# GrafikXxxxxxxYyyyyyyyyyy/StableDiffusion

Hardware: AMD Instinct MI355X
Metric: denoise-loop latents/s (512px, 50-step DDIM, batch 4) (higher is better)
Workload: dtype f16; 1 GPU; SD1.5 512x512, 50-step DDIM, batch 4/GPU, CFG on (UNet batch 8), UNet + VAE decode HIP kernels; global_batch=4, parallelism=dp1

## Files before the change

include/sd_engine.h:

```cpp
#ifndef SD_ENGINE_H
#define SD_ENGINE_H

#include <stdint.h>

#ifdef __cplusplus
extern "C" {
#endif

#define SD_OK 0
#define SD_ERR_INVALID 1
#define SD_ERR_STATE 2
#define SD_ERR_HIP 3
#define SD_ERR_UNSUPPORTED 4

#define SD_DTYPE_F16 0
#define SD_DTYPE_F32 1

#define SD_MAX_BLOCKS 4

typedef struct sd_unet_config {
    int32_t in_channels;
    int32_t out_channels;
    int32_t num_blocks;
    int32_t block_out_channels[SD_MAX_BLOCKS];
// ... 205 lines not shown

int sd_probe_mfma(int iters, float* tflops, void* stream);
int sd_probe_copy(int64_t bytes, int iters, float* gbs, void* stream);
int sd_probe_lds_dma(int64_t region_bytes, int passes, int depth, int shared, float* gbs, void* stream);

int sd_igemm_force(int variant, int splits);
int sd_igemm_plan(const int* geom, const int* flags, int64_t* out, char* name);

int sd_op_conv2d(const void* x_nhwc, const void* w_oihw, const void* bias, const void* rowadd,
                 const void* res_nhwc, void* y_nhwc, int N, int H, int W, int Cin, int Cout,
                 int ksize, int stride, int upsample2x, int geglu, void* stream);
int sd_op_conv2d_ex(const void* x_nhwc, const void* w_oihw, const void* bias, const void* rowadd,
                    const void* res_nhwc, void* y_nhwc, int N, int H, int W, int Cin, int Cout, int ksize,
                    int stride, int upsample2x, int geglu, int64_t ldx, int64_t ldres, int64_t ldy, int pad, int act,
                    float acc_scale, float bias_scale, int gn_groups, int* ran, void* stream);
int sd_op_conv3x3_small_cout(const void* x_nhwc, const void* w_oihw, const void* bias, void* y_nchw, int N, int H,
                             int W, int Cin, int Cout, void* stream);
int sd_op_conv2d_groupnorm(const void* x_nhwc, const void* w_oihw, const void* bias, const void* rowadd,
                           const void* res_nhwc, void* y_conv_nhwc, const void* gamma, const void* beta,
                           void* y_gn_nhwc, int N, int H, int W, int Cin, int Cout, int ksize, int stride,
                           int upsample2x, int groups, float eps, int silu, int* stats_from_epilogue, void* stream);
int sd_op_groupnorm_conv2d(const void* x_nhwc, const void* gamma, const void* beta, int groups, float eps, int silu,
                           const void* w_oihw, const void* bias, const void* rowadd, const void* res_nhwc, void* y_nhwc,
                           int N, int H, int W, int Cin, int Cout, int ksize, int iters, float* ms_per_launch, int* fused,
                           void* stream);
int sd_op_unet_conv_in(const void* x_nchw, const void* w_oihw, const void* bias, void* y_nhwc, float* gn_summaries, int groups,
                       int N, int Cin, int H, int W, int Cout, int iters, float* ms_per_launch, void* stream);
int sd_op_unet_conv_out(const void* x_nhwc, const void* gamma, const void* beta, int groups, float eps, int silu,
                        const void* w_oihw, const void* bias, void* y_nchw, int N, int H, int W, int C, int Cout, int iters,
                        float* ms_per_launch, void* stream);
// ... 79 lines not shown
```

stablediffusion_amd/_lib.py:

```python
from __future__ import annotations

import ctypes as C
import os

_HERE = os.path.dirname(os.path.abspath(__file__))
LIB_PATH = os.path.join(_HERE, "libsd_engine.so")

SD_MAX_BLOCKS = 4
SD_STEP_MAX_SLOTS = 4
SD_STEP_MAX_WRITES = 2
SD_DTYPE_F16 = 0
SD_DTYPE_F32 = 1


class SdUNetConfig(C.Structure):
    _fields_ = [
        ("in_channels", C.c_int32),
        ("out_channels", C.c_int32),
        ("num_blocks", C.c_int32),
        ("block_out_channels", C.c_int32 * SD_MAX_BLOCKS),
        ("down_block_has_attn", C.c_int32 * SD_MAX_BLOCKS),
        ("up_block_has_attn", C.c_int32 * SD_MAX_BLOCKS),
        ("num_heads", C.c_int32 * SD_MAX_BLOCKS),
        ("transformer_layers", C.c_int32 * SD_MAX_BLOCKS),
# ... 172 lines not shown
    "sd_images_to_uint8": (_I, [_P, _P, _I, _I, _I, _I, _P]),
    "sd_cfg_linear_step": (_I, [_P, _P, _P, _I64, _F, _F, _F, _F, _F, _F, _P]),
    "sd_cfg_rescale_linear_step": (_I, [_P, _P, _P, _I, _I64, _F, _F, _F, _F, _F, _F, _F, _P, _P]),
    "sd_lcm_step": (_I, [_P, _I, _P, _P, _P, _I64, _F, _F, _F, _F, _F, _P]),
    "sd_sched_affine_step": (_I, [_P, _I, _P, _P, _P, _I64, _I64, _F, C.POINTER(SdStepPlan), _P]),
    "sd_igemm_force": (_I, [_I, _I]),
    "sd_igemm_plan": (_I, [C.POINTER(_I), C.POINTER(_I), C.POINTER(_I64), C.c_char_p]),
    "sd_probe_mfma": (_I, [_I, C.POINTER(_F), _P]),
    "sd_probe_lds_dma": (_I, [_I64, _I, _I, _I, C.POINTER(_F), _P]),
    "sd_probe_copy": (_I, [_I64, _I, C.POINTER(_F), _P]),
    "sd_prof_enable": (_I, [_I]),
    "sd_prof_collect": (_I, [C.POINTER(SdProfEntry), _I, C.POINTER(_I)]),
    "sd_op_conv2d": (_I, [_P, _P, _P, _P, _P, _P, _I, _I, _I, _I, _I, _I, _I, _I, _I, _P]),
    "sd_op_conv2d_ex": (_I, [_P, _P, _P, _P, _P, _P, _I, _I, _I, _I, _I, _I, _I, _I, _I, _I64, _I64, _I64, _I, _I, _F, _F, _I,
                             C.POINTER(_I), _P]),
    "sd_op_conv3x3_small_cout": (_I, [_P, _P, _P, _P, _I, _I, _I, _I, _I, _P]),
    "sd_op_conv2d_groupnorm": (_I, [_P, _P, _P, _P, _P, _P, _P, _P, _P, _I, _I, _I, _I, _I, _I, _I, _I, _I, _F, _I,
                                    C.POINTER(_I), _P]),
    "sd_op_groupnorm_conv2d": (_I, [_P, _P, _P, _I, _F, _I, _P, _P, _P, _P, _P, _I, _I, _I, _I, _I, _I, _I, C.POINTER(_F),
                                    C.POINTER(_I), _P]),
    "sd_op_unet_conv_in": (_I, [_P, _P, _P, _P, _P, _I, _I, _I, _I, _I, _I, _I, C.POINTER(_F), _P]),
    "sd_op_unet_conv_out": (_I, [_P, _P, _P, _I, _F, _I, _P, _P, _P, _I, _I, _I, _I, _I, _I, C.POINTER(_F), _P]),
    "sd_op_ffn_geglu": (_I, [_P, _P, _P, _F, _P, _P, _P, _P, _P, _I, _I, _I, C.POINTER(_F), C.POINTER(_I), _P]),
    "sd_op_linear_rowstats": (_I, [_P, _P, _P, _P, _P, _P, _I, _I, _I, C.POINTER(_I), C.POINTER(_I), C.POINTER(_I), _P]),
    "sd_op_ln_linear": (_I, [_P, _P, _I, _I, _P, _P, _F, _P, _P, _P, _I, _I, _I, _I, _I, _F, C.POINTER(_I), _P]),
    "sd_op_ln_ffn_geglu": (_I, [_P, _P, _I, _I, _P, _P, _F, _P, _P, _P, _P, _P, _I, _I, C.POINTER(_I), _P]),
    "sd_op_fold_linear": (_I, [_P, _P, _P, _P, _P, _P, _I, _I, _I, _P]),
    "sd_op_ffn_geglu_proj_out": (_I, [_P, _P, _P, _P, _F, _P, _P, _P, _P, _P, _P, _P, _P, C.POINTER(_I), _I, _I, _I,
                                      C.POINTER(_I), _P]),
    "sd_bench_conv2d": (_I, [_P, _P, _P, _I, _I, _I, _I, _I, _I, _I, _I, _I, _I, C.POINTER(_F), _P]),
# ... 61 lines not shown
```

stablediffusion_amd/csrc/capi.cpp:

```cpp
#include <cmath>
#include <cstdio>
#include <new>

#include "model.h"
#include <cstdlib>

using namespace sd;

struct sd_unet { UNet impl; explicit sd_unet(const sd_unet_config& c) : impl(c) {} };
struct sd_vae { VAE impl; explicit sd_vae(const sd_vae_config& c) : impl(c) {} };
struct sd_clip { CLIP impl; explicit sd_clip(const sd_clip_config& c) : impl(c) {} };
struct sd_clip_vision { CLIPVision impl; explicit sd_clip_vision(const sd_clip_vision_config& c) : impl(c) {} };
struct sd_controlnet {
    ControlNet impl;
    sd_controlnet(const sd_unet_config& c, int cc) : impl(c, cc) {}
};
struct sd_ip_adapter {
    IPAdapter impl;
    sd_ip_adapter(const sd_unet_config& c, const sd_ip_projection_config& p) : impl(c, p) {}
    ~sd_ip_adapter() { if (impl.attached) impl.attached->set_ip_adapter(nullptr); }
};

namespace {

// ... 1690 lines not shown
    WeightStore ws;
    const int64_t so[2] = {O, J}, si[2] = {J, K}, sbo[1] = {O}, sbi[1] = {J};
    ws.declare("o.weight", {O, J}); ws.declare("o.bias", {O});
    ws.declare("i.weight", {J, K}); ws.declare("i.bias", {J});
    int rc;
    if ((rc = ws.set("o.weight", w_outer, so, 2, 0)) || (rc = ws.set("o.bias", b_outer, sbo, 1, 1)) ||
        (rc = ws.set("i.weight", w_inner, si, 2, 0)) || (rc = ws.set("i.bias", b_inner, sbi, 1, 1))) return rc;
    ConvW f;
    if ((rc = ws.fold_linear("o", "i", &f))) return rc;
    SD_HIP_CHECK(hipMemcpy(w_folded, f.w, (size_t)O * f.K * sizeof(half_t), hipMemcpyDeviceToDevice));
    SD_HIP_CHECK(hipMemcpy(b_folded, f.bias, (size_t)O * sizeof(float), hipMemcpyDeviceToDevice));
    SD_HIP_CHECK(hipDeviceSynchronize());
    return SD_OK;
}

int sd_op_ffn_geglu_proj_out(const void* x_in, const void* t3, const void* ln_gamma, const void* ln_beta, float ln_eps,
                             const void* w1, const void* b1, const void* w2, const void* b2, const void* w_po,
                             const void* b_po, void* y, float* gn_summaries, int* gn_rows, int M, int C, int imgs, int* fused,
                             void* stream) {
    if (!x_in || !t3 || !ln_gamma || !ln_beta || !w1 || !b1 || !w2 || !b2 || !w_po || !b_po || !y || M < 1 || C < 64 ||
        C % 64 != 0 || imgs < 1 || M % imgs != 0 || ln_eps != 1e-5f) {
        set_error("sd_op_ffn_geglu_proj_out: bad arguments (C % 64, M % imgs, ln_eps = 1e-5: the transformer's)"); return SD_ERR_INVALID;
    }
    hipStream_t s = static_cast<hipStream_t>(stream);
    SD_HIP_CHECK(hipStreamSynchronize(s));
    const int G = 32;
    WeightStore ws;
    const int64_t C8 = 8L * C, C4 = 4L * C;
    const int64_t s1[2] = {C8, C}, s2[2] = {C, C4}, so[2] = {C, C}, sc[1] = {C}, s8[1] = {C8};
    ws.declare("norm3.weight", {C}); ws.declare("norm3.bias", {C});
// ... 50 lines not shown
```

stablediffusion_amd/csrc/engine.h:

```cpp
#pragma once
#include <map>
#include <string>
#include <unordered_map>
#include <vector>

#include "kernels.h"

namespace sd {

struct View {
    half_t* p = nullptr;
    long ld = 0;
    int C = 0;
    View() {}
    View(half_t* p_, long ld_, int C_) : p(p_), ld(ld_), C(C_) {}
    View slice(int c0, int c) const { return View(p + c0, ld, c); }
};

class Arena {
  public:
    ~Arena();
    int reserve(size_t bytes);
    void begin(bool dry) { dry_ = dry; off_ = 0; if (dry) peak_ = 0; }
    void* alloc(size_t bytes);
// ... 6 lines not shown
    bool dry() const { return dry_; }
    bool overflow() const { return overflow_; }

  private:
    char* base_ = nullptr;
    size_t cap_ = 0, off_ = 0, peak_ = 0;
    bool dry_ = false, overflow_ = false;
};

struct ConvW {
    half_t* w = nullptr;
    float* bias = nullptr;
    int cin = 0, cout = 0, ks = 1;
    long K = 0;
    float* wsum = nullptr;
};
struct RowStat {
    float* p = nullptr;
    int parts = 0;
    int width = 0;
};
struct GnStatBuf {
    float* buf = nullptr;
    GnStats st;
};
struct ConvFuse {
    const RowStat* ln_in = nullptr;
    float ln_eps = 0.f;
    RowStat* stat_out = nullptr;
    GnStatBuf* gn_out = nullptr;
    int gn_groups = 0;
    const struct NormW* gn_in = nullptr;
    GnStats gn_in_stats;
    int gn_in_groups = 0;
    float gn_in_eps = 0.f;
    int gn_in_silu = 0;
    float acc_scale = 1.f, bias_scale = 1.f;
    int tile_variant = -1, tile_splits = 0;
};
struct NormW {
    float* gamma = nullptr;
    float* beta = nullptr;
    float* gb = nullptr;
    int C = 0;
};

struct RawTensor {
    std::vector<int64_t> shape;
    half_t* dev = nullptr;
    long numel = 0;
};

class WeightStore {
  public:
    ~WeightStore();
    void declare(const std::string& key, std::vector<int64_t> shape);
    int set(const std::string& key, const void* data, const int64_t* shape, int ndim, int dtype);
    bool complete(std::string* missing) const;
    const RawTensor* raw(const std::string& key) const;
    int pack_conv(const std::string& prefix, ConvW* out, bool has_bias = true);
    int pack_rows(const std::vector<std::string>& weight_keys, const std::vector<std::string>& bias_keys,
                  ConvW* out);
    int pack_geglu(const std::string& prefix, ConvW* out);
    int pack_norm(const std::string& prefix, NormW* out);
    int fold_ln(ConvW* w, const NormW& ln, int rows_scaled, float row_scale);
    int fold_linear(const std::string& outer, const std::string& inner, ConvW* out);
    void free_raw();
    void* dmalloc(size_t bytes);
    int64_t packed_bytes() const { return packed_bytes_; }

    std::vector<std::string> order;
    std::unordered_map<std::string, RawTensor> tensors;

  private:
    int host_floats(const std::string& key, std::vector<float>* out) const;
// ... 48 lines not shown
```

stablediffusion_amd/csrc/igemm2.hip:

```cpp
#include <atomic>
#include <cstdlib>
#include <mutex>

#include "kernels.h"

namespace sd {
namespace {

constexpr int BK = 64;
constexpr int kMaxLnParts = 20;
template <int N>
__device__ __forceinline__ void wait_vmcnt() {
    static_assert(N >= 0 && N <= 63, "vmcnt is a 6-bit field");
    asm volatile("s_waitcnt vmcnt(%0)" ::"n"(N) : "memory");
}
template <int PER, int YMAX>
__device__ __forceinline__ void wait_stages(int y) {
    if constexpr (YMAX == 0) {
        wait_vmcnt<0>();
    } else {
        if (y >= YMAX) wait_vmcnt<PER * YMAX>();
        else wait_stages<PER, YMAX - 1>(y);
    }
}
// ... 975 lines not shown
}

template <int BN>
int launch_halo(const IGemmParams& p, float* partial, int splits, hipStream_t s) {
    if (p.gni_part) {
        if (p.gni_groups < 1 || p.gni_groups > 32 || 512 % p.gni_groups != 0 || p.Cin % p.gni_groups != 0 || !p.gni_gb) {
            set_error("conv3x3_halo_kernel: fused GroupNorm needs 1..32 groups dividing 512 and the packed affine");
            return 1;
        }
        return launch_halo_t<BN, true, false>(p, partial, splits, s);
    }
    if constexpr (BN == 160) {
        if (p.gnstat_out && splits <= 1) return launch_halo_t<BN, false, false>(p, partial, splits, s);
    }
    return launch_halo_t<BN, false, true>(p, partial, splits, s);
}

template <int BM, int BN, int WM, int WN, int STAGES, bool PW, bool STAG, int BKT>
int launch_v2p(const IGemmParams& p, float* partial, int splits, hipStream_t s) {
    constexpr size_t lds = IGemm2Lds<BM, BN, STAGES, BKT>::TOTAL;
    static_assert(lds <= 160 * 1024, "LDS budget");
    static PerDeviceOnce attr_once;
    if (attr_once.first()) {
        SD_HIP_CHECK(hipFuncSetAttribute(reinterpret_cast<const void*>(&igemm2_kernel<BM, BN, WM, WN, STAGES, PW, STAG, BKT>),
                                         hipFuncAttributeMaxDynamicSharedMemorySize, (int)lds));
    }
    const int tiles = cdiv(p.M, BM) * cdiv(p.Cout, BN);
    const int nk = p.K / BKT;
    const int per = cdiv(nk, splits);
    const int eff_splits = cdiv(nk, per);
// ... 192 lines not shown
    }
    route();
    pl.variant = v;
    pl.splits = sp;
    pl.partial_floats = sp > 1 ? (long)sp * p.M * p.Cout : 0;
    if (p.geglu && (!is_ws(v) || pg_k320) && !forced && pgemm_geglu_supported(p)) pl.kind = kKindPgemmGeglu;
    else if ((v == kReg || (kVariants[v].reg_alt && g3_auto && !forced)) && sp <= 1 && igemm3_supported(p)) pl.kind = kReg;
    else pl.kind = v == kReg ? kRegFallback : v;
    const Variant& t = kVariants[pl.kind == kKindPgemmGeglu ? v : pl.kind];
    pl.bm = t.bm; pl.bn = t.bn;
    if (pl.kind == kKindPgemmGeglu) snprintf(pl.name, sizeof(pl.name), "geglu_persist_kernel");
    else snprintf(pl.name, sizeof(pl.name), t.name, p.KS == 1 && p.stride == 1 && p.up == 0 ? "true" : "false");
    return pl;
}

IGemmLaunchNote igemm2_last_launch() { return t_note; }

int igemm2_max_ln_parts() { return kMaxLnParts; }

int launch_igemm2(const IGemmParams& p, float* partial, hipStream_t s, const IGemmPlan* plan) {
    t_note = IGemmLaunchNote();
    if (p.ln_stat && (p.ln_parts < 1 || p.ln_parts > kMaxLnParts)) {
        set_error("igemm2: ln_parts " + std::to_string(p.ln_parts) + " outside 1.." + std::to_string(kMaxLnParts) +
                  " (row-statistics parts a folded LayerNorm reads per row)");
        return 1;
    }
    IGemmParams q = p;
    IGemmPlan own;
    if (!plan || (plan->splits > 1 && !partial)) {
        q.rowstat_out = nullptr; q.gnstat_out = nullptr;
// ... 11 lines not shown
```

stablediffusion_amd/csrc/kernels.h:

```cpp
#pragma once
#include "common.h"

namespace sd {

struct IGemmParams {
    const half_t* x; long ldx;
    const half_t* w;
    const float* bias;
    const float* rowadd; int rowadd_ld;
    const half_t* res; long ldres;
    half_t* y; long ldy;
    int N, H, W, Cin;
    int OH, OW, Cout;
    int KS, stride, pad, up;
    int M, K;
    int geglu;
    int mfast = 0;
    int act = 0;
    float* rowstat_out = nullptr;
    int rowstat_parts = 0;
    const float* ln_stat = nullptr;
    int ln_parts = 0, ln_C = 0, ln_part_w = 0;
    float ln_eps = 0.f;
    const float* ln_wsum = nullptr;
// ... 28 lines not shown
struct IGemmPlan {
    int kind = kKindIgemm1;
    int variant = -1;
    int splits = 1;
    long partial_floats = 0;
    int bm = 0, bn = 0;
    bool rowstats = false;
    int rs_parts = 1, rs_part_w = 0;
    bool gnstats = false;
    int gn_rows = 0;
    bool scales_ok = false;
    char name[64] = "";
};
IGemmPlan igemm2_plan(IGemmParams& p, const IGemmRequest& rq = IGemmRequest());
int launch_igemm2(const IGemmParams& p, float* partial, hipStream_t s, const IGemmPlan* plan = nullptr);
int igemm2_max_ln_parts();
struct IGemmLaunchNote {
    int splits = 1;
    int reducer = 0;
};
IGemmLaunchNote igemm2_last_launch();
bool igemm3_supported(const IGemmParams& p);
int launch_igemm3(const IGemmParams& p, int mfast, hipStream_t s);
constexpr int kWeightRowPad = 256;
bool wsgemm_supported(const IGemmParams& p);
int wsgemm_rowstat_parts(const IGemmParams& p);
int launch_wsgemm(const IGemmParams& p, hipStream_t s);
bool pgemm_geglu_supported(const IGemmParams& p);
int launch_pgemm_geglu(const IGemmParams& p, hipStream_t s);

// ... 184 lines not shown
```

stablediffusion_amd/csrc/misc.hip:

```cpp
#include <cstdint>
#include <cstdlib>
#include <map>
#include <mutex>
#include <utility>

#include "kernels.h"

namespace sd {
namespace {

__device__ __forceinline__ void sinusoid_pair(float t, int f, int half, float shift, float* sn, float* cs) {
    const float freq = __expf(-9.210340371976184f * (float)f / ((float)half - shift));
    const float ang = t * freq;
    sincosf(ang, sn, cs);
}

__global__ void sinusoid_kernel(const float* __restrict__ t, int t_stride, float* __restrict__ out, int count,
                                int dim, int flip, float shift, long out_ld) {
    const int half = dim >> 1;
    const int i = blockIdx.x * blockDim.x + threadIdx.x;
    if (i >= count * half) return;
    const int b = i / half, f = i - b * half;
    float sn, cs;
    sinusoid_pair(t[(long)b * t_stride], f, half, shift, &sn, &cs);
// ... 203 lines not shown
    if (kq < (long)KH * KW * I) {
        int ci, tap;
        if (I % 64 == 0) {
            const int slab = (int)(kq >> 6), cl = (int)(kq & 63);
            const int cs = slab / (KH * KW);
            tap = slab - cs * (KH * KW);
            ci = cs * 64 + cl;
        } else {
            ci = (int)(kq % I);
            tap = (int)(kq / I);
        }
        const int kh = tap / KW, kw = tap - kh * KW;
        val = w[((o * I + ci) * KH + kh) * KW + kw];
    }
    wp[i] = val;
}

__global__ void cfg_duplicate_kernel(const half_t* __restrict__ lat, half_t* __restrict__ out, long n,
                                     float scale) {
    const long i = (long)blockIdx.x * blockDim.x + threadIdx.x;
    if (i >= n) return;
    const half_t v = (half_t)((float)lat[i] * scale);
    out[i] = v;
    out[n + i] = v;
}
constexpr int RD_PER_THREAD = 4;
constexpr int RD_UNITS = 256 * RD_PER_THREAD;
struct RowDupDev {
    const uint4* src[kRowDupMax];
    uint4* dst[kRowDupMax];
// ... 652 lines not shown
    SD_HIP_CHECK(hipGetLastError());
    return 0;
}
int launch_conv3x3_small_cout(const half_t* x, long ldx, const half_t* w, long K, const float* bias, half_t* y_nchw,
                              int N, int H, int W, int Cin, int Cout, hipStream_t s) {
    if (Cout < 1 || Cout > 4 || Cin % 64 != 0 || K != 9L * Cin) { set_error("conv3x3_small_cout: Cout in 1..4, Cin % 64 == 0"); return 1; }
    const long tiles = (long)N * ((H + CO_TH - 1) / CO_TH) * ((W + CO_TW - 1) / CO_TW);
    if (tiles == 0) return 0;
    hipLaunchKernelGGL(conv3x3_small_cout_kernel<4>, dim3((unsigned)tiles), dim3(256), 0, s, x, ldx, w, K, bias, y_nchw, N, H, W,
                       Cin, Cout);
    SD_HIP_CHECK(hipGetLastError());
    return 0;
}
int launch_pack_conv(const half_t* w, half_t* wp, int O, int I, int KH, int KW, long Kpad, hipStream_t s) {
    hipLaunchKernelGGL(pack_conv_kernel, grid1d((long)O * Kpad), dim3(256), 0, s, w, wp, O, I, KH, KW, Kpad);
    SD_HIP_CHECK(hipGetLastError());
    return 0;
}
int launch_cfg_duplicate(const half_t* lat, half_t* out, long n, float scale, hipStream_t s) {
    hipLaunchKernelGGL(cfg_duplicate_kernel, grid1d(n), dim3(256), 0, s, lat, out, n, scale);
    SD_HIP_CHECK(hipGetLastError());
    return 0;
}
int launch_row_dup(const RowDupSeg* segs, int count, hipStream_t s) {
    if (count < 0 || count > kRowDupMax) { set_error("row_dup: too many segments"); return 1; }
    RowDupDev p;
    int blocks = 0, k = 0;
    for (int i = 0; i < count; ++i) {
        const RowDupSeg& g = segs[i];
        if (g.rows <= 0 || g.row_bytes <= 0) continue;
// ... 174 lines not shown
```

stablediffusion_amd/csrc/runtime.cpp:

```cpp
#include "engine.h"

#include <atomic>
#include <cstdio>
#include <mutex>
#include <cstdlib>
#include <cstring>

namespace sd {

static thread_local std::string g_last_error;
void set_error(const std::string& msg) { g_last_error = msg; }
const std::string& last_error() { return g_last_error; }

Arena::~Arena() {
    if (base_) (void)hipFree(base_);
}

int Arena::reserve(size_t bytes) {
    if (bytes <= cap_) return 0;
    if (base_) { (void)hipFree(base_); base_ = nullptr; cap_ = 0; }
    SD_HIP_CHECK(hipMalloc(reinterpret_cast<void**>(&base_), bytes));
    cap_ = bytes;
    return 0;
}
// ... 93 lines not shown
    return 0;
}

static long round_up(long a, long b) { return (a + b - 1) / b * b; }

static int upload_bias(WeightStore* ws, const std::vector<float>& host, int cout, float** dst) {
    const long padded = round_up(cout, kWeightRowPad);
    std::vector<float> buf((size_t)padded, 0.f);
    std::memcpy(buf.data(), host.data(), (size_t)cout * sizeof(float));
    *dst = static_cast<float*>(ws->dmalloc((size_t)padded * sizeof(float)));
    if (!*dst) { set_error("hipMalloc failed (bias)"); return 3; }
    SD_HIP_CHECK(hipMemcpy(*dst, buf.data(), (size_t)padded * sizeof(float), hipMemcpyHostToDevice));
    return 0;
}

int WeightStore::pack_conv(const std::string& prefix, ConvW* out, bool has_bias) {
    const RawTensor* w = raw(prefix + ".weight");
    if (!w) { set_error("missing weight: " + prefix + ".weight"); return 2; }
    const int O = (int)w->shape[0], I = (int)w->shape[1];
    const int KH = w->shape.size() == 4 ? (int)w->shape[2] : 1;
    const int KW = w->shape.size() == 4 ? (int)w->shape[3] : 1;
    const long K = round_up((long)KH * KW * I, 64);
    const long rows = round_up(O, kWeightRowPad);
    out->cin = I; out->cout = O; out->ks = KH; out->K = K;
    out->w = static_cast<half_t*>(dmalloc((size_t)rows * K * sizeof(half_t)));
    if (!out->w) { set_error("hipMalloc failed (weights)"); return 3; }
    SD_HIP_CHECK(hipMemsetAsync(out->w, 0, (size_t)rows * K * sizeof(half_t), 0));
    int rc = launch_pack_conv(w->dev, out->w, O, I, KH, KW, K, 0);
    if (rc) return rc;
    out->bias = nullptr;
    if (has_bias) {
        std::vector<float> b;
        rc = host_floats(prefix + ".bias", &b);
        if (rc) return rc;
        rc = upload_bias(this, b, O, &out->bias);
        if (rc) return rc;
    }
    return 0;
}

int WeightStore::pack_rows(const std::vector<std::string>& wkeys, const std::vector<std::string>& bkeys,
                           ConvW* out) {
    long total = 0;
    int I = -1;
// ... 216 lines not shown
    p.geglu = geglu;
    p.act = act;
    if (ln_in) {
        if (!w.wsum) { set_error("op_conv: LayerNorm statistics passed to a linear without folded weights"); c.err = 1; return; }
        p.ln_stat = ln_in->p; p.ln_parts = ln_in->parts; p.ln_part_w = ln_in->width; p.ln_C = (int)w.K; p.ln_eps = ln_eps; p.ln_wsum = w.wsum;
    }
    if (fuse && fuse->gn_in) {
        p.gni_part = fuse->gn_in_stats.part; p.gni_S = fuse->gn_in_stats.S; p.gni_rows = fuse->gn_in_stats.rows;
        p.gni_groups = fuse->gn_in_groups; p.gni_eps = fuse->gn_in_eps; p.gni_silu = fuse->gn_in_silu;
        p.gni_gb = fuse->gn_in->gb;
        if (c.dry) p.gni_part = reinterpret_cast<const float*>(8);
    }
    if (fuse && (fuse->acc_scale != 1.f || fuse->bias_scale != 1.f)) { p.acc_scale = fuse->acc_scale; p.bias_scale = fuse->bias_scale; }
    IGemmRequest rq{stat_out ? stat_out->p : nullptr, gn_out ? gn_out->buf : nullptr, fuse ? fuse->gn_groups : 0};
    if (fuse) { rq.hint_variant = fuse->tile_variant; rq.hint_splits = fuse->tile_splits; }
    const IGemmPlan plan = igemm2_plan(p, rq);
    const bool v2 = plan.kind != kKindIgemm1;
    if ((p.acc_scale != 1.f || p.bias_scale != 1.f) && !plan.scales_ok) { set_error("op_conv: output scaling needs the LDS-DMA kernels (not GEGLU / weight-stationary)"); c.err = 1; return; }
    if (ln_in && !v2) { set_error("op_conv: the LayerNorm fold needs the LDS-DMA kernel"); c.err = 1; return; }
    if (act && !v2) { set_error("op_conv: activation epilogue needs the LDS-DMA kernel (Cin % 64, Cout % 8)"); c.err = 1; return; }
    if (gn_out) {
        gn_out->st = GnStats();
        if (plan.gnstats) { gn_out->st.part = gn_out->buf; gn_out->st.rows = plan.gn_rows; gn_out->st.S = p.OH * p.OW / plan.gn_rows; }
    }
    const bool own_stats = plan.rowstats;
    if (stat_out) { stat_out->parts = plan.rs_parts; stat_out->width = plan.rs_part_w; }
    float* partial = plan.partial_floats > 0 ? c.arena->alloc_f(plan.partial_floats) : nullptr;
    if (c.dry || c.err) return;
    if (prof_enabled()) {
        const double kreal = (double)w.ks * w.ks * w.cin;
// ... 149 lines not shown
```

stablediffusion_amd/csrc/unet.cpp:

```cpp
#include <algorithm>
#include <vector>

#include "model.h"
#include <cmath>
#include <cstdlib>

namespace sd {

void declare_resnet(WeightStore& ws, const std::string& p, int cin, int cout, int temb) {
    ws.declare(p + ".norm1.weight", {cin});
    ws.declare(p + ".norm1.bias", {cin});
    ws.declare(p + ".conv1.weight", {cout, cin, 3, 3});
    ws.declare(p + ".conv1.bias", {cout});
    if (temb) {
        ws.declare(p + ".time_emb_proj.weight", {cout, temb});
        ws.declare(p + ".time_emb_proj.bias", {cout});
    }
    ws.declare(p + ".norm2.weight", {cout});
    ws.declare(p + ".norm2.bias", {cout});
    ws.declare(p + ".conv2.weight", {cout, cout, 3, 3});
    ws.declare(p + ".conv2.bias", {cout});
    if (cin != cout) {
        ws.declare(p + ".conv_shortcut.weight", {cout, cin, 1, 1});
        ws.declare(p + ".conv_shortcut.bias", {cout});
// ... 223 lines not shown
    temb_total = 0;
    kv_total = 0;
    kv_keys.clear();
    if ((rc = pack_encoder(&tw, &tb))) return rc;
    up_res.assign((size_t)nb, {}); up_att.assign((size_t)nb, {}); up_us.assign((size_t)nb, ConvW());
    for (int i = 0; i < nb; ++i) {
        const std::string p = "up_blocks." + std::to_string(i);
        up_res[i].resize((size_t)cfg.layers_per_block + 1);
        if (cfg.up_block_has_attn[i]) up_att[i].resize((size_t)cfg.layers_per_block + 1);
        for (int j = 0; j < cfg.layers_per_block + 1; ++j) {
            if ((rc = pack_resnet(p + ".resnets." + std::to_string(j), &up_res[i][j], &tw, &tb))) return rc;
            if (cfg.up_block_has_attn[i] &&
                (rc = pack_xformer(p + ".attentions." + std::to_string(j), &up_att[i][j], cfg.num_heads[nb - 1 - i],
                                   cfg.transformer_layers[nb - 1 - i]))) return rc;
        }
        if (i != nb - 1 && (rc = ws.pack_conv(p + ".upsamplers.0.conv", &up_us[i]))) return rc;
    }
    if ((rc = ws.pack_norm("conv_norm_out", &norm_out))) return rc;
    if ((rc = ws.pack_conv("conv_out", &conv_out))) return rc;
    if ((rc = ws.pack_rows(tw, tb, &temb_stack))) return rc;
    if (!kv_keys.empty() && (rc = ws.pack_rows(kv_keys, {}, &kv_all))) return rc;
    kv_keys.clear();
    SD_HIP_CHECK(hipDeviceSynchronize());
    ws.free_raw();
    finalized = true;
    return 0;
}

std::vector<std::pair<std::string, int>> unet_xattn_sites(const sd_unet_config& cfg, bool mid_last) {
    const int nb = cfg.num_blocks;
    const int* boc = cfg.block_out_channels;
// ... 1071 lines not shown
```

stablediffusion_amd/csrc/vae.cpp:

```cpp
#include "model.h"
#include <cmath>

namespace sd {

void declare_resnet(WeightStore& ws, const std::string& p, int cin, int cout, int temb);

namespace {
constexpr float kVaeEps = 1e-6f;

void declare_attn(WeightStore& ws, const std::string& p, int c) {
    ws.declare(p + ".group_norm.weight", {c});
    ws.declare(p + ".group_norm.bias", {c});
    for (const char* n : {"to_q", "to_k", "to_v", "to_out.0"}) {
        ws.declare(p + "." + n + ".weight", {c, c});
        ws.declare(p + "." + n + ".bias", {c});
    }
}
}

VAE::VAE(const sd_vae_config& c) : cfg(c) {
    const int nb = cfg.num_blocks;
    const int* boc = cfg.block_out_channels;
    const int lc = cfg.latent_channels;
    ws.declare("encoder.conv_in.weight", {boc[0], cfg.in_channels, 3, 3});
// ... 84 lines not shown
    std::string missing;
    if (!ws.complete(&missing)) { set_error("finalize: weight not set: " + missing); return 2; }
    const int nb = cfg.num_blocks;
    int rc;
    if ((rc = pack_pointwise("post_quant_conv", &pq_w, &pq_b))) return rc;
    if ((rc = ws.pack_conv("decoder.conv_in", &d_conv_in))) return rc;
    if ((rc = pack_resnet("decoder.mid_block.resnets.0", &d_mid0))) return rc;
    if ((rc = pack_attn("decoder.mid_block.attentions.0", &d_attn))) return rc;
    if ((rc = pack_resnet("decoder.mid_block.resnets.1", &d_mid1))) return rc;
    d_up.assign((size_t)nb, {}); d_us.assign((size_t)nb, ConvW());
    for (int i = 0; i < nb; ++i) {
        const std::string p = "decoder.up_blocks." + std::to_string(i);
        d_up[i].resize((size_t)cfg.layers_per_block + 1);
        for (int j = 0; j < cfg.layers_per_block + 1; ++j)
            if ((rc = pack_resnet(p + ".resnets." + std::to_string(j), &d_up[i][j]))) return rc;
        if (i != nb - 1 && (rc = ws.pack_conv(p + ".upsamplers.0.conv", &d_us[i]))) return rc;
    }
    if ((rc = ws.pack_norm("decoder.conv_norm_out", &d_norm_out))) return rc;
    if ((rc = ws.pack_conv("decoder.conv_out", &d_conv_out))) return rc;
    if ((rc = pack_pointwise("quant_conv", &q_w, &q_b))) return rc;
    if ((rc = ws.pack_conv("encoder.conv_in", &e_conv_in))) return rc;
    e_down.assign((size_t)nb, {}); e_ds.assign((size_t)nb, ConvW());
    for (int i = 0; i < nb; ++i) {
        const std::string p = "encoder.down_blocks." + std::to_string(i);
        e_down[i].resize((size_t)cfg.layers_per_block);
        for (int j = 0; j < cfg.layers_per_block; ++j)
            if ((rc = pack_resnet(p + ".resnets." + std::to_string(j), &e_down[i][j]))) return rc;
        if (i != nb - 1 && (rc = ws.pack_conv(p + ".downsamplers.0.conv", &e_ds[i]))) return rc;
    }
    if ((rc = pack_resnet("encoder.mid_block.resnets.0", &e_mid0))) return rc;
    if ((rc = pack_attn("encoder.mid_block.attentions.0", &e_attn))) return rc;
// ... 215 lines not shown
```

Baseline: 7.878 latents/s.

## Fold nearest-2x upsample into per-parity 2x2 convolution weights

Precomputes four folded 2x2 weight sets (one per output parity) for upsampler 3x3 convs and adds a halo-based MFMA kernel that convolves the low-resolution input directly, writing interleaved high-res output. This removes the 9/4 redundant MACs and the upsampled-input traffic of conv-after-nearest-upsample. It adds extra weight memory, a new kernel with its own GN-stat epilogue, and shape restrictions; unsupported shapes fall back to the old path. The folded weights are summed in fp32 and stored as f16, which can change rounding slightly.

Result: faster. 8.033 latents/s, median of 6 (+2.0%).

```diff
diff --git a/include/sd_engine.h b/include/sd_engine.h
--- a/include/sd_engine.h
+++ b/include/sd_engine.h
@@ -243,6 +243,11 @@
                     const void* res_nhwc, void* y_nhwc, int N, int H, int W, int Cin, int Cout, int ksize,
                     int stride, int upsample2x, int geglu, int64_t ldx, int64_t ldres, int64_t ldy, int pad, int act,
                     float acc_scale, float bias_scale, int gn_groups, int* ran, void* stream);
+int sd_upconv_fold_supported(int N, int H, int W, int Cin, int Cout);
+int sd_op_fold_upconv(const void* w_oihw, void* out, int Cout, int Cin, void* stream);
+int sd_op_upconv2x_ex(const void* x_nhwc, const void* w_oihw, const void* bias, const void* rowadd, const void* res_nhwc,
+                      void* y_nhwc, int N, int H, int W, int Cin, int Cout, int64_t ldx, int64_t ldres, int64_t ldy,
+                      float acc_scale, float bias_scale, int gn_groups, float* gn_summaries, int* ran, void* stream);
 int sd_op_conv3x3_small_cout(const void* x_nhwc, const void* w_oihw, const void* bias, void* y_nchw, int N, int H,
                              int W, int Cin, int Cout, void* stream);
 int sd_op_conv2d_groupnorm(const void* x_nhwc, const void* w_oihw, const void* bias, const void* rowadd,
diff --git a/stablediffusion_amd/_lib.py b/stablediffusion_amd/_lib.py
--- a/stablediffusion_amd/_lib.py
+++ b/stablediffusion_amd/_lib.py
@@ -210,6 +210,10 @@
     "sd_op_conv2d": (_I, [_P, _P, _P, _P, _P, _P, _I, _I, _I, _I, _I, _I, _I, _I, _I, _P]),
     "sd_op_conv2d_ex": (_I, [_P, _P, _P, _P, _P, _P, _I, _I, _I, _I, _I, _I, _I, _I, _I, _I64, _I64, _I64, _I, _I, _F, _F, _I,
                              C.POINTER(_I), _P]),
+    "sd_upconv_fold_supported": (_I, [_I, _I, _I, _I, _I]),
+    "sd_op_fold_upconv": (_I, [_P, _P, _I, _I, _P]),
+    "sd_op_upconv2x_ex": (_I, [_P, _P, _P, _P, _P, _P, _I, _I, _I, _I, _I, _I64, _I64, _I64, _F, _F, _I, _P,
+                               C.POINTER(_I), _P]),
     "sd_op_conv3x3_small_cout": (_I, [_P, _P, _P, _P, _I, _I, _I, _I, _I, _P]),
     "sd_op_conv2d_groupnorm": (_I, [_P, _P, _P, _P, _P, _P, _P, _P, _P, _I, _I, _I, _I, _I, _I, _I, _I, _I, _F, _I,
                                     C.POINTER(_I), _P]),
diff --git a/stablediffusion_amd/csrc/capi.cpp b/stablediffusion_amd/csrc/capi.cpp
--- a/stablediffusion_amd/csrc/capi.cpp
+++ b/stablediffusion_amd/csrc/capi.cpp
@@ -1728,6 +1728,83 @@
     return SD_OK;
 }
 
+int sd_upconv_fold_supported(int N, int H, int W, int Cin, int Cout) {
+    return upconv_fold_supported(N, H, W, Cin, Cout, Cin) ? 1 : 0;
+}
+
+int sd_op_fold_upconv(const void* w_oihw, void* out, int Cout, int Cin, void* stream) {
+    if (!w_oihw || !out || Cout < 1 || Cin < 64 || Cin % 64 != 0) {
+        set_error("sd_op_fold_upconv: bad arguments (Cin must be a multiple of 64)"); return SD_ERR_INVALID;
+    }
+    hipStream_t s = static_cast<hipStream_t>(stream);
+    const long rows = ((long)Cout + kWeightRowPad - 1) / kWeightRowPad * kWeightRowPad, K4 = 4L * Cin;
+    DevScope scope;
+    half_t* wp = nullptr;
+    SD_DEV_ALLOC(scope, wp, (size_t)4 * rows * K4 * sizeof(half_t));
+    SD_HIP_CHECK(hipMemsetAsync(wp, 0, (size_t)4 * rows * K4 * sizeof(half_t), s));
+    if (int rc = launch_fold_upconv(static_cast<const half_t*>(w_oihw), wp, Cout, Cin, s)) return rc;
+    for (int par = 0; par < 4; ++par)
+        SD_HIP_CHECK(hipMemcpyAsync(static_cast<half_t*>(out) + (long)par * Cout * K4, wp + (long)par * rows * K4,
+                                    (size_t)Cout * K4 * sizeof(half_t), hipMemcpyDeviceToDevice, s));
+    SD_HIP_CHECK(hipStreamSynchronize(s));
+    return SD_OK;
+}
+
+int sd_op_upconv2x_ex(const void* x, const void* w_oihw, const void* bias_f32, const void* rowadd_f32, const void* res,
+                      void* y, int N, int H, int W, int Cin, int Cout, int64_t ldx, int64_t ldres, int64_t ldy,
+                      float acc_scale, float bias_scale, int gn_groups, float* gn_summaries, int* ran, void* stream) {
+    if (!x || !w_oihw || !y || !ran || N < 1 || H < 1 || W < 1 || Cin < 64 || Cin % 64 != 0 || Cout < 1 || gn_groups < 0 ||
+        !(acc_scale > 0.f) || !(bias_scale > 0.f)) {
+        set_error("sd_op_upconv2x_ex: bad arguments (Cin % 64 == 0, positive scales)"); return SD_ERR_INVALID;
+    }
+    auto ld_ok = [](int64_t ld, int dense) { return ld == dense || (ld > dense && ld % 8 == 0); };
+    if (!ld_ok(ldx, Cin) || !ld_ok(ldy, Cout) || (res && !ld_ok(ldres, Cout))) {
+        set_error("sd_op_upconv2x_ex: ldx / ldres / ldy must be the dense width or a wider multiple of 8"); return SD_ERR_INVALID;
+    }
+    for (int i = 0; i < 4; ++i) ran[i] = 0;
+    hipStream_t s = static_cast<hipStream_t>(stream);
+    const long K = 9L * Cin, rows = ((long)Cout + kWeightRowPad - 1) / kWeightRowPad * kWeightRowPad;
+    DevScope scope;
+    ConvW cw;
+    cw.cin = Cin; cw.cout = Cout; cw.ks = 3; cw.K = K;
+    SD_DEV_ALLOC(scope, cw.w, (size_t)rows * K * sizeof(half_t));
+    SD_DEV_ALLOC(scope, cw.bias, (size_t)rows * sizeof(float));
+    SD_HIP_CHECK(hipMemsetAsync(cw.w, 0, (size_t)rows * K * sizeof(half_t), s));
+    SD_HIP_CHECK(hipMemsetAsync(cw.bias, 0, (size_t)rows * sizeof(float), s));
+    int rc = launch_pack_conv(static_cast<const half_t*>(w_oihw), cw.w, Cout, Cin, 3, 3, K, s);
+    if (rc) return rc;
+    if (bias_f32) SD_HIP_CHECK(hipMemcpyAsync(cw.bias, bias_f32, (size_t)Cout * sizeof(float), hipMemcpyDeviceToDevice, s));
+    if (Cout % 8 == 0) {
+        SD_DEV_ALLOC(scope, cw.w_up, (size_t)16 * rows * Cin * sizeof(half_t));
+        SD_HIP_CHECK(hipMemsetAsync(cw.w_up, 0, (size_t)16 * rows * Cin * sizeof(half_t), s));
+        if ((rc = launch_fold_upconv(static_cast<const half_t*>(w_oihw), cw.w_up, Cout, Cin, s))) return rc;
+    }
+    const long OHW = 4L * H * W;
+    GnStatBuf gb;
+    if (gn_groups > 0) SD_DEV_ALLOC(scope, gb.buf, (size_t)gnstat_floats(N, OHW, gn_groups) * sizeof(float));
+    int folded = 0;
+    rc = run_op_on_arena(s, 0, nullptr, [&](Ctx& c) {
+        ConvFuse f;
+        f.acc_scale = acc_scale; f.bias_scale = bias_scale;
+        f.gn_out = gn_groups > 0 ? &gb : nullptr; f.gn_groups = gn_groups;
+        f.fold_ran = &folded;
+        const View rv(const_cast<half_t*>(static_cast<const half_t*>(res)), ldres, Cout);
+        op_conv(c, cw, View(const_cast<half_t*>(static_cast<const half_t*>(x)), ldx, Cin), N, H, W,
+                View(static_cast<half_t*>(y), ldy, Cout), 1, 1, static_cast<const float*>(rowadd_f32), Cout, res ? &rv : nullptr,
+                0, -1, 0, &f);
+    });
+    if (rc) return rc;
+    ran[0] = folded;
+    if (gb.st.part) {
+        ran[1] = gb.st.S; ran[2] = (int)gb.st.rows;
+        if (gn_summaries)
+            SD_HIP_CHECK(hipMemcpyAsync(gn_summaries, gb.st.part, (size_t)N * gb.st.S * gn_groups * 2 * sizeof(float),
+                                        hipMemcpyDeviceToDevice, s));
+    }
+    SD_HIP_CHECK(hipStreamSynchronize(s));
+    return SD_OK;
+}
+
 int sd_op_ffn_geglu_proj_out(const void* x_in, const void* t3, const void* ln_gamma, const void* ln_beta, float ln_eps,
                              const void* w1, const void* b1, const void* w2, const void* b2, const void* w_po,
                              const void* b_po, void* y, float* gn_summaries, int* gn_rows, int M, int C, int imgs, int* fused,
diff --git a/stablediffusion_amd/csrc/engine.h b/stablediffusion_amd/csrc/engine.h
--- a/stablediffusion_amd/csrc/engine.h
+++ b/stablediffusion_amd/csrc/engine.h
@@ -44,6 +44,7 @@
     int cin = 0, cout = 0, ks = 1;
     long K = 0;
     float* wsum = nullptr;
+    half_t* w_up = nullptr;
 };
 struct RowStat {
     float* p = nullptr;
@@ -67,6 +68,7 @@
     int gn_in_silu = 0;
     float acc_scale = 1.f, bias_scale = 1.f;
     int tile_variant = -1, tile_splits = 0;
+    int* fold_ran = nullptr;
 };
 struct NormW {
     float* gamma = nullptr;
@@ -88,7 +90,7 @@
     int set(const std::string& key, const void* data, const int64_t* shape, int ndim, int dtype);
     bool complete(std::string* missing) const;
     const RawTensor* raw(const std::string& key) const;
-    int pack_conv(const std::string& prefix, ConvW* out, bool has_bias = true);
+    int pack_conv(const std::string& prefix, ConvW* out, bool has_bias = true, bool fold_up2x = false);
     int pack_rows(const std::vector<std::string>& weight_keys, const std::vector<std::string>& bias_keys,
                   ConvW* out);
     int pack_geglu(const std::string& prefix, ConvW* out);
diff --git a/stablediffusion_amd/csrc/igemm2.hip b/stablediffusion_amd/csrc/igemm2.hip
--- a/stablediffusion_amd/csrc/igemm2.hip
+++ b/stablediffusion_amd/csrc/igemm2.hip
@@ -1013,6 +1013,243 @@
         if (p.gnstat_out && splits <= 1) return launch_halo_t<BN, false, false>(p, partial, splits, s);
     }
     return launch_halo_t<BN, false, true>(p, partial, splits, s);
+}
+
+template <int BN>
+__global__ __launch_bounds__(512) void conv3x3_halo_up2x2_kernel(IGemmParams p) {
+#if defined(__HIP_DEVICE_COMPILE__)
+    static_assert(BN == 160 || BN == 128, "column tile");
+    constexpr unsigned kOOB = 0x80000000u;
+    constexpr int BM = 256, NW = 8, NT = 512, WAVES_N = 2;
+    constexpr int WTM = 64, WTN = BN / 2, TM = 4, TN = WTN / 16;
+    constexpr int B_INSTR = BN / 8, B_PW = (B_INSTR + NW - 1) / NW, B_REM = B_INSTR % NW;
+    constexpr int B_STAGE_HALVES = BN * 64;
+    constexpr int AJ = 7;
+    constexpr int LDC = BN + 8;
+    extern __shared__ __attribute__((aligned(16))) char smem[];
+    const int W = p.W, HW = p.H * p.W;
+    const int OW = p.OW, OHW = p.OH * p.OW;
+    const int Wt = halo_patch_width(p.H, W), Wp = Wt + 2;
+    const int R = BM / Wt;
+    const int HP = (R + 2) * Wp;
+    const int A_HALVES = HP * 64;
+    half_t* sA = reinterpret_cast<half_t*>(smem);
+    half_t* sB = sA + 2 * A_HALVES;
+    half_t* sC = reinterpret_cast<half_t*>(smem);
+
+    const int tid = threadIdx.x, lane = tid & 63;
+    const int wave = __builtin_amdgcn_readfirstlane(tid >> 6);
+    const int wm = wave / WAVES_N, wn = wave % WAVES_N;
+    const int tiles_n = (p.Cout + BN - 1) / BN, cols = 4 * tiles_n;
+    const int bid = xcd_remap(blockIdx.x, gridDim.x);
+    int tm, tc;
+    if (p.mfast) {
+        const int tiles_m = gridDim.x / cols;
+        tc = bid / tiles_m; tm = bid - tc * tiles_m;
+    } else {
+        tm = bid / cols; tc = bid - tm * cols;
+    }
+    const int par = tc / tiles_n, tn = tc - par * tiles_n;
+    const int dy = par >> 1, dx = par & 1;
+    const int n0 = tn * BN;
+    const int patches_w = W / Wt, patches = (p.H / R) * patches_w;
+    const int img = tm / patches, pidx = tm - img * patches;
+    const int row0 = (pidx / patches_w) * R, col0 = (pidx % patches_w) * Wt;
+    auto row_of = [&](int ml) {
+        const int r = ml / Wt;
+        return img * OHW + (2 * (row0 + r) + dy) * OW + 2 * (col0 + (ml - r * Wt)) + dx;
+    };
+    const int nslab = p.Cin / 64;
+
+    const long x_bytes = (long)p.N * HW * p.ldx * 2;
+    __amdgpu_buffer_rsrc_t rx = __builtin_amdgcn_make_buffer_rsrc(const_cast<half_t*>(p.x), 0, (int)x_bytes, 0x00020000);
+    const long wrows = ((long)p.Cout + kWeightRowPad - 1) / kWeightRowPad * kWeightRowPad;
+    __amdgpu_buffer_rsrc_t rw = __builtin_amdgcn_make_buffer_rsrc(const_cast<half_t*>(p.w) + (long)par * wrows * p.K, 0,
+                                                                  (int)(wrows * p.K * 2), 0x00020000);
+
+    const int NI = (HP * 8 + 63) >> 6;
+    int a_off[AJ];
+#pragma unroll
+    for (int j = 0; j < AJ; ++j) {
+        const int i = wave + NW * j;
+        const int slot = i * 64 + lane;
+        const int hp = slot >> 3, cpos = slot & 7;
+        const int hr = hp / Wp, hc = hp - hr * Wp;
+        const int ih = row0 - 1 + hr, iw = col0 - 1 + hc;
+        const bool inb = ((unsigned)ih < (unsigned)p.H) & ((unsigned)iw < (unsigned)W);
+        const int chunk = cpos ^ (hp & 7);
+        int off = -1;
+        if (i < NI && slot < HP * 8)
+            off = inb ? (int)((((long)img * HW + (long)ih * W + iw) * p.ldx + chunk * 8) * 2) : -2;
+        a_off[j] = off;
+    }
+    auto issueA = [&](int bufi, int slab) {
+        half_t* dst = sA + bufi * A_HALVES;
+#pragma unroll
+        for (int j = 0; j < AJ; ++j) {
+            const int i = wave + NW * j;
+            if (i < NI && a_off[j] != -1) {
+                const unsigned voff = a_off[j] >= 0 ? (unsigned)a_off[j] + (unsigned)(slab * 128) : kOOB;
+                __builtin_amdgcn_raw_ptr_buffer_load_lds(rx, (__attribute__((address_space(3))) void*)(dst + i * 512), 16,
+                                                         voff, 0, 0, 0);
+            }
+        }
+    };
+    const int lrow = lane >> 3;
+    const int chunkB = (lane & 7) ^ lrow;
+    const bool b_hi = B_REM == 0 || wave < B_REM;
+    const int b_cnt = b_hi ? B_PW : B_PW - 1;
+    const int b_first = b_hi ? wave * B_PW : B_REM * B_PW + (wave - B_REM) * (B_PW - 1);
+    unsigned b_off[B_PW];
+#pragma unroll
+    for (int j = 0; j < B_PW; ++j)
+        b_off[j] = (unsigned)((((long)(n0 + (b_first + j) * 8 + lrow)) * p.K + chunkB * 8) * 2);
+    auto issueB = [&](int stage, int g) {
+        half_t* dst = sB + stage * B_STAGE_HALVES;
+#pragma unroll
+        for (int j = 0; j < B_PW; ++j)
+            if (j < b_cnt)
+                __builtin_amdgcn_raw_ptr_buffer_load_lds(rw, (__attribute__((address_space(3))) void*)(dst + (b_first + j) * 512),
+                                                         16, b_off[j] + (unsigned)(g * 128), 0, 0, 0);
+    };
+
+    f4 acc[TM][TN];
+#pragma unroll
+    for (int i = 0; i < TM; ++i)
+#pragma unroll
+        for (int j = 0; j < TN; ++j) acc[i][j] = f4{0.f, 0.f, 0.f, 0.f};
+
+    const int fr = lane & 15, fq = lane >> 4;
+    int hp0[TM];
+#pragma unroll
+    for (int i = 0; i < TM; ++i) {
+        const int ml = wm * WTM + i * 16 + fr;
+        const int r = ml / Wt, c = ml - r * Wt;
+        hp0[i] = (r + dy) * Wp + c + dx;
+    }
+
+    issueA(0, 0);
+    issueB(0, 0);
+    issueB(1, 1);
+    int g = 0, st = 0, abuf = 0;
+    bool a_next = false;
+    for (int slab = 0; slab < nslab; ++slab) {
+        const bool lastslab = slab + 1 >= nslab;
+        const half_t* cA = sA + abuf * A_HALVES;
+#pragma unroll
+        for (int tap = 0; tap < 4; ++tap, ++g) {
+            if (lastslab && tap == 3) wait_vmcnt<0>();
+            else if (a_next && (tap == 1 || tap == 2)) wait_vmcnt<7>();
+            else wait_vmcnt<2>();
+            __builtin_amdgcn_s_barrier();
+            const int st2 = st >= 1 ? st - 1 : 2;
+            if (!(lastslab && tap >= 2)) issueB(st2, g + 2);
+            if (tap == 0) {
+                a_next = !lastslab;
+                if (a_next) issueA(abuf ^ 1, slab + 1);
+            }
+            const half_t* cB = sB + st * B_STAGE_HALVES;
+            const int tapoff = (tap >> 1) * Wp + (tap & 1);
+#pragma unroll
+            for (int ks = 0; ks < 2; ++ks) {
+                h8 fa[TM], fb[TN];
+                const int ch = ks * 4 + fq;
+#pragma unroll
+                for (int i = 0; i < TM; ++i) {
+                    const int hp = hp0[i] + tapoff;
+                    fa[i] = *reinterpret_cast<const h8*>(cA + hp * 64 + ((ch ^ (hp & 7)) << 3));
+                }
+#pragma unroll
+                for (int j = 0; j < TN; ++j) {
+                    const int r = wn * WTN + j * 16 + fr;
+                    fb[j] = *reinterpret_cast<const h8*>(cB + r * 64 + ((ch ^ (r & 7)) << 3));
+                }
+#pragma unroll
+                for (int i = 0; i < TM; ++i)
+#pragma unroll
+                    for (int j = 0; j < TN; ++j)
+                        acc[i][j] = __builtin_amdgcn_mfma_f32_16x16x32_f16(fb[j], fa[i], acc[i][j], 0, 0, 0);
+            }
+            st = st == 2 ? 0 : st + 1;
+        }
+        abuf ^= 1;
+    }
+
+    __syncthreads();
+    const float acc_scale = *reinterpret_cast<const volatile float*>(&p.acc_scale);
+    const float bias_scale = *reinterpret_cast<const volatile float*>(&p.bias_scale);
+    {
+        f4 add[TN];
+#pragma unroll
+        for (int j = 0; j < TN; ++j)
+            add[j] = p.bias ? *reinterpret_cast<const f4*>(p.bias + n0 + wn * WTN + j * 16 + fq * 4) * bias_scale : f4{0.f, 0.f, 0.f, 0.f};
+#pragma unroll
+        for (int i = 0; i < TM; ++i) {
+            const int pr = wm * WTM + i * 16 + fr;
+#pragma unroll
+            for (int j = 0; j < TN; ++j) {
+                const int col = wn * WTN + j * 16 + fq * 4;
+                const f4 v = acc[i][j] * acc_scale + add[j];
+                h4 o = {(half_t)v[0], (half_t)v[1], (half_t)v[2], (half_t)v[3]};
+                *reinterpret_cast<h4*>(sC + pr * LDC + col) = o;
+            }
+        }
+    }
+    __syncthreads();
+    constexpr int CH = BN / 8;
+    constexpr int RPP = NT / CH;
+    constexpr int ITER = (BM + RPP - 1) / RPP;
+    const int c8 = tid % CH, rr = tid / CH;
+    const int c = c8 * 8, n = n0 + c;
+    const bool okc = rr < RPP && n < p.Cout;
+    const int cpg = p.gnstat_out ? p.Cout / p.gn_groups : 8;
+    const int g_first = n / cpg;
+    const int gsplit = (g_first + 1) * cpg - n;
+    float gm0 = 0.f, gq0 = 0.f, gm1 = 0.f, gq1 = 0.f;
+    float gp0 = 0.f, gp1 = 0.f;
+    int gnv = 0;
+#pragma unroll
+    for (int it = 0; it < ITER; ++it) {
+        const int r = rr + it * RPP;
+        if (okc && r < BM) {
+            const h8 v = *reinterpret_cast<const h8*>(sC + r * LDC + c);
+            *reinterpret_cast<h8*>(p.y + (long)row_of(r) * p.ldy + n) = v;
+            if (p.gnstat_out) { gn_chunk_accum(v, gsplit, it == 0, gp0, gp1, gm0, gq0, gm1, gq1); ++gnv; }
+        }
+    }
+    if (p.gnstat_out) {
+        float* sG = reinterpret_cast<float*>(smem + ((BM * LDC * 2 + 15) & ~15));
+        gn_part_finish(gsplit, gnv, gp0, gp1, gm0, gq0, gm1, gq1);
+        gn_tile_stats<BM, BN, NT>(sG, tid, gm0, gq0, gm1, gq1, n0, p.Cout, cpg, p.gn_groups,
+                                  p.gnstat_out + (((long)img * patches + pidx) * 4 + par) * p.gn_groups * 2);
+    }
+#endif
+}
+
+template <int BN>
+int launch_up2x2_t(const IGemmParams& p, hipStream_t s) {
+    const int Wt = halo_patch_width(p.H, p.W), R = 256 / Wt;
+    size_t lds = (size_t)2 * (R + 2) * (Wt + 2) * 128 + (size_t)3 * BN * 128;
+    const size_t epi = (size_t)256 * (BN + 8) * 2 + 16 + 512 * 16;
+    if (lds < epi) lds = epi;
+    if (lds > 160 * 1024) { set_error("conv3x3_halo_up2x2_kernel: LDS budget"); return 1; }
+    static size_t attr_by_dev[64] = {};
+    static std::mutex attr_mu;
+    int dev = 0;
+    (void)hipGetDevice(&dev);
+    std::lock_guard<std::mutex> attr_lock(attr_mu);
+    size_t& attr = attr_by_dev[dev & 63];
+    if (lds > attr) {
+        SD_HIP_CHECK(hipFuncSetAttribute(reinterpret_cast<const void*>(&conv3x3_halo_up2x2_kernel<BN>),
+                                         hipFuncAttributeMaxDynamicSharedMemorySize, (int)lds));
+        attr = lds;
+    }
+    const int blocks = p.N * (p.H * p.W / 256) * 4 * cdiv(p.Cout, BN);
+    IGemmParams q = p;
+    q.mfast = weights_outweigh_activations(p);
+    hipLaunchKernelGGL((conv3x3_halo_up2x2_kernel<BN>), dim3(blocks), dim3(512), lds, s, q);
+    SD_HIP_CHECK(hipGetLastError());
+    return 0;
 }
 
 template <int BM, int BN, int WM, int WN, int STAGES, bool PW, bool STAG, int BKT>
@@ -1235,6 +1472,40 @@
     return pl;
 }
 
+bool upconv_fold_supported(int N, int H, int W, int Cin, int Cout, long ldx) {
+    static const bool off = getenv("SD_NO_UPCONV_FOLD") != nullptr;
+    if (off || N < 1 || H < 1 || W < 1 || Cin < 64 || Cout < 8) return false;
+    const long wrows = ((long)Cout + kWeightRowPad - 1) / kWeightRowPad * kWeightRowPad;
+    return Cin % 64 == 0 && Cout % 8 == 0 && halo_patch_width(H, W) > 0 && (long)N * H * W * ldx * 2 < (1L << 31) &&
+           wrows * 4 * Cin * 2 < (1L << 31) && (long)N * H * W * 4 < (1L << 31);
+}
+
+UpconvFoldPlan upconv_fold_plan(IGemmParams& p, const half_t* w_fold, const IGemmRequest& rq) {
+    UpconvFoldPlan pl;
+    if (!w_fold || p.up != 1 || p.KS != 3 || p.stride != 1 || p.pad != 1 || p.OH != 2 * p.H || p.OW != 2 * p.W ||
+        p.K != 9 * p.Cin || p.geglu || p.act || p.rowadd || p.res || p.ln_stat || p.gni_part || rq.rowstat ||
+        !upconv_fold_supported(p.N, p.H, p.W, p.Cin, p.Cout, p.ldx))
+        return pl;
+    pl.ok = true;
+    pl.bn = p.Cout % 160 == 0 ? 160 : 128;
+    p.w = w_fold; p.K = 4 * p.Cin; p.KS = 2;
+    const int G = rq.gn_groups, cpg = G > 0 && p.Cout % G == 0 ? p.Cout / G : 0;
+    p.gnstat_out = nullptr; p.gn_groups = 0;
+    if (rq.gnstat && (cpg >= 8 || cpg == 4) && (pl.bn % cpg == 0 || p.Cout <= pl.bn)) {
+        p.gnstat_out = rq.gnstat; p.gn_groups = G;
+        pl.gnstats = true; pl.gn_rows = 256;
+    }
+    snprintf(pl.name, sizeof(pl.name), "conv3x3_halo_kernel<%d>/up2x2", pl.bn);
+    return pl;
+}
+
+int launch_upconv_fold(const IGemmParams& p, const UpconvFoldPlan& plan, hipStream_t s) {
+    if (!plan.ok || p.KS != 2 || p.K != 4 * p.Cin || halo_patch_width(p.H, p.W) == 0) {
+        set_error("launch_upconv_fold: not a folded-upsample problem (upconv_fold_plan decides)"); return 1;
+    }
+    return plan.bn == 160 ? launch_up2x2_t<160>(p, s) : launch_up2x2_t<128>(p, s);
+}
+
 IGemmLaunchNote igemm2_last_launch() { return t_note; }
 
 int igemm2_max_ln_parts() { return kMaxLnParts; }
diff --git a/stablediffusion_amd/csrc/kernels.h b/stablediffusion_amd/csrc/kernels.h
--- a/stablediffusion_amd/csrc/kernels.h
+++ b/stablediffusion_amd/csrc/kernels.h
@@ -66,6 +66,17 @@
 };
 IGemmPlan igemm2_plan(IGemmParams& p, const IGemmRequest& rq = IGemmRequest());
 int launch_igemm2(const IGemmParams& p, float* partial, hipStream_t s, const IGemmPlan* plan = nullptr);
+bool upconv_fold_supported(int N, int H, int W, int Cin, int Cout, long ldx);
+struct UpconvFoldPlan {
+    bool ok = false;
+    int bn = 0;
+    bool gnstats = false;
+    int gn_rows = 0;
+    char name[64] = "";
+};
+UpconvFoldPlan upconv_fold_plan(IGemmParams& p, const half_t* w_fold, const IGemmRequest& rq);
+int launch_upconv_fold(const IGemmParams& p, const UpconvFoldPlan& plan, hipStream_t s);
+int launch_fold_upconv(const half_t* w_oihw, half_t* wp, int O, int I, hipStream_t s);
 int igemm2_max_ln_parts();
 struct IGemmLaunchNote {
     int splits = 1;
diff --git a/stablediffusion_amd/csrc/misc.hip b/stablediffusion_amd/csrc/misc.hip
--- a/stablediffusion_amd/csrc/misc.hip
+++ b/stablediffusion_amd/csrc/misc.hip
@@ -241,6 +241,25 @@
         val = w[((o * I + ci) * KH + kh) * KW + kw];
     }
     wp[i] = val;
+}
+
+__global__ void fold_upconv_kernel(const half_t* __restrict__ w, half_t* __restrict__ wp, int O, int I, long rows) {
+    const long K4 = 4L * I;
+    const long i = (long)blockIdx.x * blockDim.x + threadIdx.x;
+    if (i >= 4 * O * K4) return;
+    const long kq = i % K4;
+    const long o = (i / K4) % O;
+    const int par = (int)(i / (K4 * O));
+    const int dy = par >> 1, dx = par & 1;
+    const int slab = (int)(kq >> 6), cl = (int)(kq & 63);
+    const int tap = slab & 3, a = tap >> 1, b = tap & 1;
+    const long ci = (long)(slab >> 2) * 64 + cl;
+    const int h_lo = a == 0 ? 0 : 2 - (1 - dy), h_hi = a == 0 ? dy : 2;
+    const int w_lo = b == 0 ? 0 : 2 - (1 - dx), w_hi = b == 0 ? dx : 2;
+    float s = 0.f;
+    for (int kh = h_lo; kh <= h_hi; ++kh)
+        for (int kw = w_lo; kw <= w_hi; ++kw) s += (float)w[((o * I + ci) * 3 + kh) * 3 + kw];
+    wp[((long)par * rows + o) * K4 + kq] = (half_t)s;
 }
 
 __global__ void cfg_duplicate_kernel(const half_t* __restrict__ lat, half_t* __restrict__ out, long n,
@@ -923,6 +942,13 @@
 }
 int launch_pack_conv(const half_t* w, half_t* wp, int O, int I, int KH, int KW, long Kpad, hipStream_t s) {
     hipLaunchKernelGGL(pack_conv_kernel, grid1d((long)O * Kpad), dim3(256), 0, s, w, wp, O, I, KH, KW, Kpad);
+    SD_HIP_CHECK(hipGetLastError());
+    return 0;
+}
+int launch_fold_upconv(const half_t* w, half_t* wp, int O, int I, hipStream_t s) {
+    if (O < 1 || I < 64 || I % 64 != 0) { set_error("fold_upconv: Cin must be a multiple of 64"); return 1; }
+    const long rows = ((long)O + kWeightRowPad - 1) / kWeightRowPad * kWeightRowPad;
+    hipLaunchKernelGGL(fold_upconv_kernel, grid1d(16L * O * I), dim3(256), 0, s, w, wp, O, I, rows);
     SD_HIP_CHECK(hipGetLastError());
     return 0;
 }
diff --git a/stablediffusion_amd/csrc/runtime.cpp b/stablediffusion_amd/csrc/runtime.cpp
--- a/stablediffusion_amd/csrc/runtime.cpp
+++ b/stablediffusion_amd/csrc/runtime.cpp
@@ -131,7 +131,7 @@
     return 0;
 }
 
-int WeightStore::pack_conv(const std::string& prefix, ConvW* out, bool has_bias) {
+int WeightStore::pack_conv(const std::string& prefix, ConvW* out, bool has_bias, bool fold_up2x) {
     const RawTensor* w = raw(prefix + ".weight");
     if (!w) { set_error("missing weight: " + prefix + ".weight"); return 2; }
     const int O = (int)w->shape[0], I = (int)w->shape[1];
@@ -145,6 +145,14 @@
     SD_HIP_CHECK(hipMemsetAsync(out->w, 0, (size_t)rows * K * sizeof(half_t), 0));
     int rc = launch_pack_conv(w->dev, out->w, O, I, KH, KW, K, 0);
     if (rc) return rc;
+    out->w_up = nullptr;
+    if (fold_up2x && KH == 3 && KW == 3 && I % 64 == 0 && O % 8 == 0) {
+        const size_t bytes = (size_t)4 * rows * 4 * I * sizeof(half_t);
+        out->w_up = static_cast<half_t*>(dmalloc(bytes));
+        if (!out->w_up) { set_error("hipMalloc failed (folded upsample weights)"); return 3; }
+        SD_HIP_CHECK(hipMemsetAsync(out->w_up, 0, bytes, 0));
+        if ((rc = launch_fold_upconv(w->dev, out->w_up, O, I, 0))) return rc;
+    }
     out->bias = nullptr;
     if (has_bias) {
         std::vector<float> b;
@@ -391,6 +399,32 @@
     if (fuse && (fuse->acc_scale != 1.f || fuse->bias_scale != 1.f)) { p.acc_scale = fuse->acc_scale; p.bias_scale = fuse->bias_scale; }
     IGemmRequest rq{stat_out ? stat_out->p : nullptr, gn_out ? gn_out->buf : nullptr, fuse ? fuse->gn_groups : 0};
     if (fuse) { rq.hint_variant = fuse->tile_variant; rq.hint_splits = fuse->tile_splits; }
+    if (fuse && fuse->fold_ran) *fuse->fold_ran = 0;
+    if (up == 1 && w.w_up) {
+        const UpconvFoldPlan fp = upconv_fold_plan(p, w.w_up, rq);
+        if (fp.ok) {
+            if (gn_out) {
+                gn_out->st = GnStats();
+                if (fp.gnstats) { gn_out->st.part = gn_out->buf; gn_out->st.rows = fp.gn_rows; gn_out->st.S = p.OH * p.OW / fp.gn_rows; }
+            }
+            if (fuse && fuse->fold_ran) *fuse->fold_ran = 1;
+            if (c.dry || c.err) return;
+            if (prof_enabled()) {
+                const char* name = fp.name;
+                static const bool by_shape = getenv("SD_PROF_SHAPES") != nullptr;
+                char nbuf[64];
+                if (by_shape) {
+                    snprintf(nbuf, sizeof(nbuf), "up2x2<%d> %dx%dx%d ks%d%s", fp.bn, p.M, p.Cout, p.K, p.KS, p.gnstat_out ? " gs" : "");
+                    name = nbuf;
+                }
+                prof_open(c.stream, name, 2.0 * p.M * w.cout * 4.0 * w.cin,
+                          2.0 * ((double)N * H * W * w.cin + 16.0 * w.cout * w.cin + (double)p.M * w.cout));
+            }
+            c.err = launch_upconv_fold(p, fp, c.stream);
+            prof_close(c.stream);
+            return;
+        }
+    }
     const IGemmPlan plan = igemm2_plan(p, rq);
     const bool v2 = plan.kind != kKindIgemm1;
     if ((p.acc_scale != 1.f || p.bias_scale != 1.f) && !plan.scales_ok) { set_error("op_conv: output scaling needs the LDS-DMA kernels (not GEGLU / weight-stationary)"); c.err = 1; return; }
diff --git a/stablediffusion_amd/csrc/unet.cpp b/stablediffusion_amd/csrc/unet.cpp
--- a/stablediffusion_amd/csrc/unet.cpp
+++ b/stablediffusion_amd/csrc/unet.cpp
@@ -261,7 +261,7 @@
                 (rc = pack_xformer(p + ".attentions." + std::to_string(j), &up_att[i][j], cfg.num_heads[nb - 1 - i],
                                    cfg.transformer_layers[nb - 1 - i]))) return rc;
         }
-        if (i != nb - 1 && (rc = ws.pack_conv(p + ".upsamplers.0.conv", &up_us[i]))) return rc;
+        if (i != nb - 1 && (rc = ws.pack_conv(p + ".upsamplers.0.conv", &up_us[i], true, true))) return rc;
     }
     if ((rc = ws.pack_norm("conv_norm_out", &norm_out))) return rc;
     if ((rc = ws.pack_conv("conv_out", &conv_out))) return rc;
diff --git a/stablediffusion_amd/csrc/vae.cpp b/stablediffusion_amd/csrc/vae.cpp
--- a/stablediffusion_amd/csrc/vae.cpp
+++ b/stablediffusion_amd/csrc/vae.cpp
@@ -122,7 +122,7 @@
         d_up[i].resize((size_t)cfg.layers_per_block + 1);
         for (int j = 0; j < cfg.layers_per_block + 1; ++j)
             if ((rc = pack_resnet(p + ".resnets." + std::to_string(j), &d_up[i][j]))) return rc;
-        if (i != nb - 1 && (rc = ws.pack_conv(p + ".upsamplers.0.conv", &d_us[i]))) return rc;
+        if (i != nb - 1 && (rc = ws.pack_conv(p + ".upsamplers.0.conv", &d_us[i], true, true))) return rc;
     }
     if ((rc = ws.pack_norm("decoder.conv_norm_out", &d_norm_out))) return rc;
     if ((rc = ws.pack_conv("decoder.conv_out", &d_conv_out))) return rc;
```
